# vllm-project/production-stack

Hardware: AMD Instinct MI355X
Metric: output_tokens_per_sec (higher is better)
Workload: dtype bfloat16; 1 GPU; multi-round-qa; model=llama-3-8b, users_per_gpu=320, rounds_per_conversation=10, max_model_len=8192, parallelism=dp1, prefix_caching=True, kv_cache_dtype=auto, quantization=none

## Files before the change

csrc/attention.hip:

```cpp
#include "ps_common.h"

template <int HEAD_DIM, int GQ, int BLOCK_SIZE, int NWAVES, int LOWREG,
          typename KVT>
__global__ __launch_bounds__(NWAVES * 64, LOWREG ? 3 : 1) void paged_attn_decode_kernel(
    unsigned short* __restrict__ out,
    float* __restrict__ ws_acc,
    float* __restrict__ ws_ml,
    const unsigned short* __restrict__ q,
    const KVT* __restrict__ k_cache,
    const KVT* __restrict__ v_cache,
    const int* __restrict__ block_tables,
    const int* __restrict__ seq_lens,
    int max_blocks, float scale, int KH, long q_stride, int window) {
  using KVTr = ps_kv_traits<KVT>;
  using kvec8 = typename KVTr::vec8;
  constexpr int D = HEAD_DIM;
  constexpr int LPG = D / 8;
  constexpr int TPW = 64 / LPG;
  static_assert(BLOCK_SIZE % TPW == 0, "block size must divide");

  const int seq = blockIdx.x;
  const int kvh = blockIdx.y;
  const int ctx = seq_lens[seq];
  const int wave = threadIdx.x >> 6;
  const int lane = threadIdx.x & 63;
  const int sg = lane / LPG;
  const int sl = lane % LPG;

  ps_bf16x8 qp[GQ];
  const unsigned short* qbase = q + (long)seq * q_stride + (long)kvh * GQ * D;
#pragma unroll
  for (int g = 0; g < GQ; g++)
    qp[g] = *(const ps_bf16x8*)(qbase + g * D + sl * 8);
  float qf[GQ][8];
  if constexpr (!LOWREG) {
#pragma unroll
    for (int g = 0; g < GQ; g++)
#pragma unroll
      for (int j = 0; j < 8; j++) qf[g][j] = ps_bf16_to_f32(qp[g][j]);
  }

  float m[GQ], l[GQ], acc[GQ][8];
#pragma unroll
  for (int g = 0; g < GQ; g++) {
    m[g] = PS_NEG_INF;
    l[g] = 0.f;
#pragma unroll
    for (int j = 0; j < 8; j++) acc[g][j] = 0.f;
  }

  const int nblocks = (ctx + BLOCK_SIZE - 1) / BLOCK_SIZE;
  const int win_lo = (window > 0 && ctx > window) ? ctx - window : 0;
  const int first_block = win_lo / BLOCK_SIZE;
  const int nsplit = gridDim.z;
  const int split = blockIdx.z;
  const int live_blocks = nblocks - first_block;
  const int per_split = (live_blocks + nsplit - 1) / nsplit;
  const int b_begin = first_block + split * per_split;
  const int b_end = min(nblocks, b_begin + per_split);
  const int* bt = block_tables + (long)seq * max_blocks;
  constexpr int TPB = BLOCK_SIZE / TPW;
  for (int b = b_begin + wave; b < b_end; b += NWAVES) {
    const long blk = bt[b];
    const KVT* kb = k_cache + ((blk * KH + kvh) * BLOCK_SIZE) * D;
    const KVT* vb = v_cache + ((blk * KH + kvh) * BLOCK_SIZE) * D;
    const int valid_tokens = min(BLOCK_SIZE, ctx - b * BLOCK_SIZE);
    float sc[GQ][TPB];
    kvec8 vv[TPB];
    if constexpr (LOWREG) {
#pragma unroll
      for (int g = 0; g < GQ; g++)
        asm volatile("" : "+v"(qp[g]));
    }
#pragma unroll
    for (int tt = 0; tt < TPB; tt++) {
      const int tok = tt * TPW + sg;
      const bool valid =
          tok < valid_tokens && b * BLOCK_SIZE + tok >= win_lo;
      kvec8 kv = *(const kvec8*)(kb + tok * D + sl * 8);
      if constexpr (!LOWREG)
        vv[tt] = *(const kvec8*)(vb + tok * D + sl * 8);
      float kf[8];
      KVTr::to_f32x8(kv, kf);
#pragma unroll
      for (int g = 0; g < GQ; g++) {
        float s = 0.f;
#pragma unroll
        for (int j = 0; j < 8; j++) {
          if constexpr (LOWREG)
            s += ps_bf16_to_f32(qp[g][j]) * kf[j];
          else
            s += qf[g][j] * kf[j];
        }
        s = ps_group_sum<LPG>(s) * scale;
        sc[g][tt] = valid ? s : PS_NEG_INF;
      }
    }
    if constexpr (LOWREG) {
#pragma unroll
      for (int tt = 0; tt < TPB; tt++)
        vv[tt] = *(const kvec8*)(vb + (tt * TPW + sg) * D + sl * 8);
    }
#pragma unroll
    for (int g = 0; g < GQ; g++) {
      float bmax = sc[g][0];
#pragma unroll
      for (int tt = 1; tt < TPB; tt++) bmax = fmaxf(bmax, sc[g][tt]);
      const float mnew = fmaxf(m[g], bmax);
      const float corr = __expf(m[g] - mnew);
      float p[TPB];
      float psum = 0.f;
#pragma unroll
// ... 18 lines not shown
#pragma unroll
  for (int off = LPG; off < 64; off <<= 1) {
#pragma unroll
    for (int g = 0; g < GQ; g++) {
      const float mo = __shfl_xor(m[g], off, 64);
      const float lo = __shfl_xor(l[g], off, 64);
      const float mnew = fmaxf(m[g], mo);
      const float c1 = __expf(m[g] - mnew);
      const float c2 = __expf(mo - mnew);
#pragma unroll
      for (int j = 0; j < 8; j++) {
        const float ao = __shfl_xor(acc[g][j], off, 64);
        acc[g][j] = acc[g][j] * c1 + ao * c2;
      }
      l[g] = l[g] * c1 + lo * c2;
      m[g] = mnew;
    }
  }

  __shared__ float sm[NWAVES][GQ];
  __shared__ float slse[NWAVES][GQ];
  __shared__ float sacc[NWAVES][GQ][D];
  if (sg == 0) {
#pragma unroll
    for (int g = 0; g < GQ; g++) {
      if (sl == 0) {
        sm[wave][g] = m[g];
        slse[wave][g] = l[g];
      }
#pragma unroll
      for (int j = 0; j < 8; j++) sacc[wave][g][sl * 8 + j] = acc[g][j];
    }
  }
  __syncthreads();
  if (wave == 0 && sg == 0) {
#pragma unroll
    for (int g = 0; g < GQ; g++) {
      float M = PS_NEG_INF, L = 0.f, A[8];
#pragma unroll
      for (int j = 0; j < 8; j++) A[j] = 0.f;
#pragma unroll
      for (int wv = 0; wv < NWAVES; wv++) {
        const float mw = sm[wv][g];
        const float mnew = fmaxf(M, mw);
        const float c1 = __expf(M - mnew);
        const float c2 = __expf(mw - mnew);
        L = L * c1 + slse[wv][g] * c2;
#pragma unroll
        for (int j = 0; j < 8; j++)
          A[j] = A[j] * c1 + sacc[wv][g][sl * 8 + j] * c2;
        M = mnew;
      }
      const long head = (long)seq * KH * GQ + (long)kvh * GQ + g;
      if (nsplit == 1) {
        const float inv = L > 0.f ? 1.f / L : 0.f;
        ps_bf16x8 ov;
#pragma unroll
        for (int j = 0; j < 8; j++) ov[j] = ps_f32_to_bf16(A[j] * inv);
        *(ps_bf16x8*)(out + head * D + sl * 8) = ov;
      } else {
        float* wa = ws_acc + (head * nsplit + split) * D + sl * 8;
#pragma unroll
        for (int j = 0; j < 8; j++) wa[j] = A[j];
        if (sl == 0) {
          float* wm = ws_ml + (head * nsplit + split) * 2;
          wm[0] = M;
          wm[1] = L;
        }
      }
    }
  }
}

template <int HEAD_DIM>
__global__ __launch_bounds__(64) void paged_attn_combine_kernel(
    unsigned short* __restrict__ out,
    const float* __restrict__ ws_acc,
    const float* __restrict__ ws_ml,
    int nsplit) {
  constexpr int D = HEAD_DIM;
  constexpr int LPG = D / 8;
  const long head = blockIdx.x;
  const int sl = threadIdx.x;
  if (sl >= LPG) return;
  float M = PS_NEG_INF, L = 0.f, A[8];
#pragma unroll
  for (int j = 0; j < 8; j++) A[j] = 0.f;
  for (int s = 0; s < nsplit; s++) {
    const float mw = ws_ml[(head * nsplit + s) * 2 + 0];
    const float lw = ws_ml[(head * nsplit + s) * 2 + 1];
    const float mnew = fmaxf(M, mw);
    const float c1 = __expf(M - mnew);
    const float c2 = __expf(mw - mnew);
    const float* wa = ws_acc + (head * nsplit + s) * D + sl * 8;
#pragma unroll
    for (int j = 0; j < 8; j++) A[j] = A[j] * c1 + wa[j] * c2;
    L = L * c1 + lw * c2;
    M = mnew;
  }
  const float inv = L > 0.f ? 1.f / L : 0.f;
  ps_bf16x8 ov;
#pragma unroll
  for (int j = 0; j < 8; j++) ov[j] = ps_f32_to_bf16(A[j] * inv);
  *(ps_bf16x8*)(out + head * D + sl * 8) = ov;
}

template <int HEAD_DIM, int BLOCK_SIZE>
__global__ __launch_bounds__(64) void paged_attn_prefill_kernel(
    unsigned short* __restrict__ out,
    const unsigned short* __restrict__ q,
    const unsigned short* __restrict__ k_cache,
    const unsigned short* __restrict__ v_cache,
    const int* __restrict__ block_tables,
    const int* __restrict__ token_seq,
    const int* __restrict__ token_pos,
    int max_blocks, float scale, int KH, int GQ, long q_stride,
    int window) {
  constexpr int D = HEAD_DIM;
  constexpr int LPG = D / 8;
  constexpr int TPW = 64 / LPG;

  const int tokid = blockIdx.x;
  const int qh = blockIdx.y;
  const int kvh = qh / GQ;
  const int seq = token_seq[tokid];
  const int pos = token_pos[tokid];
  const int ctx = pos + 1;
  const int lane = threadIdx.x & 63;
  const int sg = lane / LPG;
  const int sl = lane % LPG;
  const int QH = KH * GQ;

  float qf[8];
  {
    ps_bf16x8 qv =
        *(const ps_bf16x8*)(q + (long)tokid * q_stride + (long)qh * D + sl * 8);
#pragma unroll
    for (int j = 0; j < 8; j++) qf[j] = ps_bf16_to_f32(qv[j]) * scale;
  }

  float m = PS_NEG_INF, l = 0.f, acc[8];
#pragma unroll
  for (int j = 0; j < 8; j++) acc[j] = 0.f;

  const int nblocks = (ctx + BLOCK_SIZE - 1) / BLOCK_SIZE;
  const int win_lo = (window > 0 && ctx > window) ? ctx - window : 0;
  const int* bt = block_tables + (long)seq * max_blocks;
// ... 99 lines not shown
    for (int j = 0; j < 8; j++) {
      const float f = ps_bf16_to_f32(xv[j]);
      if (f > best) {
        best = f;
        besti = i + j;
      }
    }
  }
  const int tail_start = (V / 8) * 8;
  for (int i = tail_start + threadIdx.x; i < V; i += blockDim.x) {
    const float f = ps_bf16_to_f32(row[i]);
    if (f > best) {
      best = f;
      besti = i;
    }
  }
#pragma unroll
  for (int off = 32; off > 0; off >>= 1) {
    const float ob = __shfl_xor(best, off, 64);
    const int oi = __shfl_xor(besti, off, 64);
    if (ob > best || (ob == best && oi < besti)) {
      best = ob;
      besti = oi;
    }
  }
  __shared__ float wbest[4];
  __shared__ int wbesti[4];
  const int wave = threadIdx.x >> 6;
  if ((threadIdx.x & 63) == 0) {
    wbest[wave] = best;
    wbesti[wave] = besti;
  }
  __syncthreads();
  if (threadIdx.x == 0) {
    for (int wv = 1; wv < (int)(blockDim.x >> 6); wv++) {
      if (wbest[wv] > wbest[0] ||
          (wbest[wv] == wbest[0] && wbesti[wv] < wbesti[0])) {
        wbest[0] = wbest[wv];
        wbesti[0] = wbesti[wv];
      }
    }
    out[r] = wbesti[0];
  }
}

extern "C" {

int ps_paged_attn_decode(void* out, void* ws_acc, void* ws_ml, const void* q,
                         const void* k_cache, const void* v_cache,
                         const void* block_tables, const void* seq_lens,
                         int num_seqs, int max_blocks, float scale, int KH,
                         int GQ, int head_dim, int block_size, int num_splits,
                         long q_stride, int variant, int kv_fp8,
                         int window, hipStream_t stream) {
  dim3 grid(num_seqs, KH, num_splits);
  constexpr int NW = 4;
  dim3 block(NW * 64);
#define PS_DECODE_T(HD, G, BS, LR, KVT)                                      \
  paged_attn_decode_kernel<HD, G, BS, NW, LR, KVT>                           \
      <<<grid, block, 0, stream>>>(                                          \
          (unsigned short*)out, (float*)ws_acc, (float*)ws_ml,               \
          (const unsigned short*)q, (const KVT*)k_cache,                     \
          (const KVT*)v_cache, (const int*)block_tables,                     \
          (const int*)seq_lens, max_blocks, scale, KH, q_stride, window)
#define PS_DISPATCH_DECODE(HD, G, BS)                                        \
  do {                                                                       \
    if (kv_fp8) {                                                            \
      if (variant == 1)                                                      \
        PS_DECODE_T(HD, G, BS, 1, unsigned char);                            \
      else                                                                   \
        PS_DECODE_T(HD, G, BS, 0, unsigned char);                            \
    } else {                                                                 \
      if (variant == 1)                                                      \
        PS_DECODE_T(HD, G, BS, 1, unsigned short);                           \
      else                                                                   \
        PS_DECODE_T(HD, G, BS, 0, unsigned short);                           \
    }                                                                        \
    if (num_splits > 1)                                                      \
      paged_attn_combine_kernel<HD>                                          \
          <<<dim3(num_seqs * KH * G), 64, 0, stream>>>(                      \
              (unsigned short*)out, (const float*)ws_acc,                    \
              (const float*)ws_ml, num_splits);                              \
  } while (0)
  if (head_dim == 128 && block_size == 16) {
    switch (GQ) {
      case 1: PS_DISPATCH_DECODE(128, 1, 16); return 0;
      case 2: PS_DISPATCH_DECODE(128, 2, 16); return 0;
      case 3: PS_DISPATCH_DECODE(128, 3, 16); return 0;
      case 4: PS_DISPATCH_DECODE(128, 4, 16); return 0;
      case 6: PS_DISPATCH_DECODE(128, 6, 16); return 0;
      case 7: PS_DISPATCH_DECODE(128, 7, 16); return 0;
      case 8: PS_DISPATCH_DECODE(128, 8, 16); return 0;
      default: return -1;
    }
  }
  if (head_dim == 64 && block_size == 16 && !kv_fp8) {
    switch (GQ) {
      case 1: PS_DISPATCH_DECODE(64, 1, 16); return 0;
      case 2: PS_DISPATCH_DECODE(64, 2, 16); return 0;
      case 4: PS_DISPATCH_DECODE(64, 4, 16); return 0;
      case 8: PS_DISPATCH_DECODE(64, 8, 16); return 0;
      default: return -1;
    }
  }
  return -1;
#undef PS_DECODE_T
#undef PS_DISPATCH_DECODE
}

int ps_paged_attn_prefill(void* out, const void* q, const void* k_cache,
                          const void* v_cache, const void* block_tables,
                          const void* token_seq, const void* token_pos,
                          int num_tokens, int num_q_heads, int max_blocks,
                          float scale, int KH, int GQ, int head_dim,
                          int block_size, long q_stride, int window,
                          hipStream_t stream) {
  dim3 grid(num_tokens, num_q_heads);
  dim3 block(64);
#define PS_DISPATCH_PREFILL(HD, BS)                                         \
  paged_attn_prefill_kernel<HD, BS><<<grid, block, 0, stream>>>(            \
      (unsigned short*)out, (const unsigned short*)q,                       \
      (const unsigned short*)k_cache, (const unsigned short*)v_cache,       \
      (const int*)block_tables, (const int*)token_seq,                      \
      (const int*)token_pos, max_blocks, scale, KH, GQ, q_stride, window)
  if (head_dim == 128 && block_size == 16) {
    PS_DISPATCH_PREFILL(128, 16);
    return 0;
  }
  if (head_dim == 64 && block_size == 16) {
    PS_DISPATCH_PREFILL(64, 16);
    return 0;
  }
  return -1;
#undef PS_DISPATCH_PREFILL
}
// ... 29 lines not shown
```

csrc/bindings.cpp:

```cpp
#include <hip/hip_runtime.h>
#include <torch/extension.h>

#include <c10/hip/HIPStream.h>

#include <algorithm>

extern "C" {
void ps_rms_norm(void* out, const void* x, const void* w, float eps, long T,
                 int D, hipStream_t stream);
void ps_fused_add_rms_norm(void* x, void* residual, const void* w, float eps,
                           long T, int D, hipStream_t stream);
void ps_rms_norm_fp8(void* out_q, void* out_scale, void* x, void* residual,
                     const void* w, float eps, long T, int D, int fused,
                     hipStream_t stream);
void ps_silu_and_mul_fp8(void* out_q, void* out_scale, const void* x, long T,
                         int D, hipStream_t stream);
void ps_silu_and_mul(void* out, const void* x, long T, int D,
                     hipStream_t stream);
void ps_rope(const void* positions, void* q, void* k, const void* cos_sin,
             long T, int QH, int KH, int HD, int ROT, hipStream_t stream);
void ps_fused_rope_cache(void* qkv, const void* positions, const void* cos_sin,
                         const void* slot_mapping, void* k_cache,
                         void* v_cache, long T, int QH, int KH, int HD,
                         int ROT, long qkv_stride, int BS, int kv_fp8,
                         hipStream_t stream);
int ps_paged_attn_decode(void* out, void* ws_acc, void* ws_ml, const void* q,
                         const void* k_cache, const void* v_cache,
                         const void* block_tables, const void* seq_lens,
                         int num_seqs, int max_blocks, float scale, int KH,
                         int GQ, int head_dim, int block_size, int num_splits,
                         long q_stride, int variant, int kv_fp8, int window,
                         hipStream_t stream);
int ps_prefill_mfma32_splits(int num_tiles, int KH, int GQ);
int ps_paged_attn_prefill_mfma32(void* out, void* ws_o, void* ws_ml,
                                 long q_tokens, const void* q,
                                 const void* k_cache, const void* v_cache,
                                 const void* block_tables,
                                 const void* tile_info, int num_tiles,
                                 int num_q_heads, int max_blocks,
                                 float scale, int KH, int GQ, int head_dim,
                                 long q_stride, int kv_fp8, int window,
                                 hipStream_t stream);
int ps_paged_attn_prefill_mfma(void* out, const void* q, const void* k_cache,
                               const void* v_cache, const void* block_tables,
                               const void* tile_info, int num_tiles,
                               int num_q_heads, int max_blocks, float scale,
                               int KH, int GQ, int head_dim, long q_stride,
                               int variant, int kv_fp8, int window, hipStream_t stream);
int ps_paged_attn_prefill(void* out, const void* q, const void* k_cache,
                          const void* v_cache, const void* block_tables,
                          const void* token_seq, const void* token_pos,
                          int num_tokens, int num_q_heads, int max_blocks,
                          float scale, int KH, int GQ, int head_dim,
                          int block_size, long q_stride, int window,
                          hipStream_t stream);
void ps_reshape_and_cache(const void* k, const void* v, void* k_cache,
                          void* v_cache, const void* slot_mapping, long T,
                          int KH, int HD, int BS, int kv_fp8,
                          hipStream_t stream);
void ps_greedy_sample(void* out, const void* logits, long R, int V,
                      hipStream_t stream);
void ps_kv_quant(void* out, void* scales, const void* in, long rows, int hd,
                 hipStream_t stream);
void ps_kv_dequant(void* out, const void* in, const void* scales, long rows,
                   int hd, hipStream_t stream);
int ps_skinny_gemm_splits(int M, int N, int K);
int ps_skinny_gemm(void* out_bf16, void* ws, const void* x, const void* w,
                   int M, int N, int K, long x_stride, hipStream_t stream);
int ps_gemm8p_splits(int M, int N, int K);
int ps_gemm8p(void* out_bf16, void* ws, const void* x, const void* w, int M,
              int N, int K, long x_stride, hipStream_t stream);
int ps_lora_bgmv(void* out, const void* x, const void* A, const void* B,
                 const void* scale, const void* idx, int T, int IN, int W,
                 int R, long out_stride, long x_stride, int col_off,
                 hipStream_t stream);
}

at::Tensor cachegen_encode(at::Tensor q);
at::Tensor cachegen_decode(at::Tensor blob, int64_t hd);

namespace {

hipStream_t current_stream() {
  return c10::hip::getCurrentHIPStream().stream();
}
// ... 22 lines not shown
  TORCH_CHECK(q.dim() == 3 && q.stride(2) == 1 && q.stride(1) == HD,
              "q must be [T, H, HD] with contiguous heads");
  return q.stride(0);
}

void rms_norm(at::Tensor out, at::Tensor x, at::Tensor w, double eps) {
  CHECK_GPU_BF16(out);
  CHECK_GPU_BF16(x);
  CHECK_GPU_BF16(w);
  const long T = x.numel() / x.size(-1);
  const int D = (int)x.size(-1);
  TORCH_CHECK(D % 8 == 0, "hidden dim must be a multiple of 8");
  ps_rms_norm(out.data_ptr(), x.data_ptr(), w.data_ptr(), (float)eps, T, D,
              current_stream());
}

void fused_add_rms_norm(at::Tensor x, at::Tensor residual, at::Tensor w,
                        double eps) {
  CHECK_GPU_BF16(x);
  CHECK_GPU_BF16(residual);
  CHECK_GPU_BF16(w);
  const long T = x.numel() / x.size(-1);
  const int D = (int)x.size(-1);
  TORCH_CHECK(D % 8 == 0, "hidden dim must be a multiple of 8");
  ps_fused_add_rms_norm(x.data_ptr(), residual.data_ptr(), w.data_ptr(),
                        (float)eps, T, D, current_stream());
}

void silu_and_mul(at::Tensor out, at::Tensor x) {
  CHECK_GPU_BF16(out);
  CHECK_GPU_BF16(x);
  const int D = (int)out.size(-1);
  TORCH_CHECK(x.size(-1) == 2 * D, "x last dim must be 2*out last dim");
  TORCH_CHECK(D % 8 == 0, "feature dim must be a multiple of 8");
  const long T = out.numel() / D;
  ps_silu_and_mul(out.data_ptr(), x.data_ptr(), T, D, current_stream());
}

void rotary_embedding(at::Tensor positions, at::Tensor q, at::Tensor k,
                      at::Tensor cos_sin, long head_dim) {
  CHECK_GPU_DTYPE(positions, at::kInt);
  CHECK_GPU_BF16(q);
  CHECK_GPU_BF16(k);
  CHECK_GPU_DTYPE(cos_sin, at::kFloat);
  const long T = positions.size(0);
  const int HD = (int)head_dim;
  const int ROT = (int)cos_sin.size(-1);
  const int QH = (int)(q.numel() / T / HD);
  const int KH = (int)(k.numel() / T / HD);
  ps_rope(positions.data_ptr(), q.data_ptr(), k.data_ptr(),
          cos_sin.data_ptr(), T, QH, KH, HD, ROT, current_stream());
}

void paged_attn_decode(at::Tensor out, at::Tensor q, at::Tensor k_cache,
                       at::Tensor v_cache, at::Tensor block_tables,
                       at::Tensor seq_lens, double scale, int64_t num_splits,
                       int64_t variant, int64_t window) {
  CHECK_GPU_BF16(out);
  const int kv_fp8 = cache_fp8(k_cache);
  cache_fp8(v_cache);
  CHECK_GPU_DTYPE(block_tables, at::kInt);
  CHECK_GPU_DTYPE(seq_lens, at::kInt);
  const int S = (int)q.size(0);
  const int QH = (int)q.size(1);
  const int HD = (int)q.size(2);
  const int KH = (int)k_cache.size(1);
  const int BS = (int)k_cache.size(2);
  TORCH_CHECK(QH % KH == 0, "GQA group mismatch");
  const int GQ = QH / KH;
  const int max_blocks = (int)block_tables.size(1);
  if (num_splits <= 0) {
    const int target = 2048;
    num_splits = std::min<int64_t>(
        32, std::max<int64_t>(1, target / std::max(1, S * KH)));
  }
  at::Tensor ws_acc, ws_ml;
  void *acc_p = nullptr, *ml_p = nullptr;
  if (num_splits > 1) {
    auto opts = q.options().dtype(at::kFloat);
    ws_acc = at::empty({(long)S * QH * num_splits * HD}, opts);
    ws_ml = at::empty({(long)S * QH * num_splits * 2}, opts);
    acc_p = ws_acc.data_ptr();
    ml_p = ws_ml.data_ptr();
  }
  int rc = ps_paged_attn_decode(
      out.data_ptr(), acc_p, ml_p, q.data_ptr(), k_cache.data_ptr(),
      v_cache.data_ptr(), block_tables.data_ptr(), seq_lens.data_ptr(), S,
      max_blocks, (float)scale, KH, GQ, HD, BS, (int)num_splits,
      q_row_stride(q, HD), (int)variant, kv_fp8, (int)window,
      current_stream());
  TORCH_CHECK(rc == 0, "unsupported decode config: head_dim=", HD,
              " block_size=", BS, " gqa=", GQ);
}

void paged_attn_prefill(at::Tensor out, at::Tensor q, at::Tensor k_cache,
                        at::Tensor v_cache, at::Tensor block_tables,
                        at::Tensor token_seq, at::Tensor token_pos,
                        double scale, int64_t window) {
  CHECK_GPU_BF16(out);
  CHECK_GPU_BF16(k_cache);
  CHECK_GPU_BF16(v_cache);
  CHECK_GPU_DTYPE(block_tables, at::kInt);
  CHECK_GPU_DTYPE(token_seq, at::kInt);
  CHECK_GPU_DTYPE(token_pos, at::kInt);
  const int T = (int)q.size(0);
  const int QH = (int)q.size(1);
  const int HD = (int)q.size(2);
  const int KH = (int)k_cache.size(1);
  const int BS = (int)k_cache.size(2);
  TORCH_CHECK(QH % KH == 0, "GQA group mismatch");
  const int GQ = QH / KH;
  const int max_blocks = (int)block_tables.size(1);
  int rc = ps_paged_attn_prefill(
      out.data_ptr(), q.data_ptr(), k_cache.data_ptr(), v_cache.data_ptr(),
      block_tables.data_ptr(), token_seq.data_ptr(), token_pos.data_ptr(), T,
      QH, max_blocks, (float)scale, KH, GQ, HD, BS, q_row_stride(q, HD),
      (int)window, current_stream());
  TORCH_CHECK(rc == 0, "unsupported prefill config: head_dim=", HD,
              " block_size=", BS);
}

void paged_attn_prefill_mfma(at::Tensor out, at::Tensor q,
                             at::Tensor k_cache, at::Tensor v_cache,
                             at::Tensor block_tables, at::Tensor tile_info,
                             double scale, int64_t variant, int64_t window) {
  CHECK_GPU_BF16(out);
  const int kv_fp8 = cache_fp8(k_cache);
  cache_fp8(v_cache);
  CHECK_GPU_DTYPE(block_tables, at::kInt);
  CHECK_GPU_DTYPE(tile_info, at::kInt);
  const int QH = (int)q.size(1);
  const int HD = (int)q.size(2);
  const int KH = (int)k_cache.size(1);
  TORCH_CHECK(QH % KH == 0, "GQA group mismatch");
  TORCH_CHECK(k_cache.size(2) == 16, "mfma prefill needs block_size 16");
  const int GQ = QH / KH;
  const int NT = (int)tile_info.size(0);
  int rc;
  if (variant == 5) {
    const int splits = ps_prefill_mfma32_splits(NT, KH, QH / KH);
    const long T = q.size(0);
    void *ws_o_p = nullptr, *ws_ml_p = nullptr;
    at::Tensor ws_o, ws_ml;
// ... 159 lines not shown
  TORCH_CHECK(out.size(0) == T && idx.numel() == T, "T mismatch");
  TORCH_CHECK(col_off + W <= out.size(1), "col range out of bounds");
  int rc = ps_lora_bgmv(out.data_ptr(), x.data_ptr(), A.data_ptr(),
                        B.data_ptr(), scale.data_ptr(), idx.data_ptr(), T,
                        IN, W, R, out.stride(0), x.stride(0), (int)col_off,
                        current_stream());
  TORCH_CHECK(rc == 0, "lora_bgmv unsupported (R>64?) R=", R);
}

void kv_quant(at::Tensor out, at::Tensor scales, at::Tensor in) {
  CHECK_GPU_DTYPE(out, at::kChar);
  CHECK_GPU_DTYPE(scales, at::kFloat);
  CHECK_GPU_BF16(in);
  const int hd = (int)in.size(-1);
  TORCH_CHECK(hd % 8 == 0, "row width must be multiple of 8");
  const long rows = in.numel() / hd;
  ps_kv_quant(out.data_ptr(), scales.data_ptr(), in.data_ptr(), rows, hd,
              current_stream());
}

void kv_dequant(at::Tensor out, at::Tensor in, at::Tensor scales) {
  CHECK_GPU_BF16(out);
  CHECK_GPU_DTYPE(in, at::kChar);
  CHECK_GPU_DTYPE(scales, at::kFloat);
  const int hd = (int)out.size(-1);
  const long rows = out.numel() / hd;
  ps_kv_dequant(out.data_ptr(), in.data_ptr(), scales.data_ptr(), rows, hd,
                current_stream());
}

void greedy_sample(at::Tensor out, at::Tensor logits) {
  CHECK_GPU_DTYPE(out, at::kLong);
  CHECK_GPU_BF16(logits);
  const long R = logits.size(0);
  const int V = (int)logits.size(1);
  ps_greedy_sample(out.data_ptr(), logits.data_ptr(), R, V, current_stream());
}

}

PYBIND11_MODULE(TORCH_EXTENSION_NAME, m) {
  m.def("rms_norm", &rms_norm, "RMSNorm (bf16)");
  m.def("fused_add_rms_norm", &fused_add_rms_norm,
        "Fused residual add + RMSNorm (bf16, in-place)");
  m.def("silu_and_mul", &silu_and_mul, "SiLU-and-mul (bf16)");
  m.def("rotary_embedding", &rotary_embedding,
        "Neox-style rotary embedding (bf16, in-place)");
  m.def("paged_attn_decode", &paged_attn_decode,
        "Paged attention, decode phase (bf16 KV, split-KV)",
        pybind11::arg("out"), pybind11::arg("q"), pybind11::arg("k_cache"),
        pybind11::arg("v_cache"), pybind11::arg("block_tables"),
        pybind11::arg("seq_lens"), pybind11::arg("scale"),
        pybind11::arg("num_splits") = 0, pybind11::arg("variant") = 0,
        pybind11::arg("window") = 0);
  m.def("paged_attn_prefill", &paged_attn_prefill,
        "Paged attention, chunked prefill (bf16 KV)");
  m.def("lora_bgmv", &lora_bgmv,
        "batched-grouped LoRA matvec (per-token adapter slots)");
  m.def("paged_attn_prefill_mfma", &paged_attn_prefill_mfma,
        "Paged attention, chunked prefill via MFMA tiles (head_dim 128)",
        pybind11::arg("out"), pybind11::arg("q"), pybind11::arg("k_cache"),
        pybind11::arg("v_cache"), pybind11::arg("block_tables"),
        pybind11::arg("tile_info"), pybind11::arg("scale"),
        pybind11::arg("variant") = 4, pybind11::arg("window") = 0);
  m.def("fused_rope_cache", &fused_rope_cache,
        "Fused RoPE + paged KV append on the packed qkv tensor");
  m.def("reshape_and_cache", &reshape_and_cache,
        "Append K/V for new tokens into the paged cache");
  m.def("greedy_sample", &greedy_sample, "Per-row argmax over vocab");
  m.def("kv_quant", &kv_quant, "Row-wise int8 KV quantization");
  m.def("rms_norm_fp8", &rms_norm_fp8,
        "RMSNorm (optionally fused residual add) emitting fp8 + row scales");
  m.def("silu_and_mul_fp8", &silu_and_mul_fp8,
        "SiLU-mul emitting fp8 + row scales");
  m.def("cachegen_encode", &cachegen_encode,
        "CacheGen-style adaptive range encode of int8 KV (CPU)");
  m.def("cachegen_decode", &cachegen_decode,
        "CacheGen-style range decode -> int8 (CPU)");
  m.def("gemm8p", &gemm8p,
        "8-phase deep-pipelined bf16 GEMM (out = x @ w.T)");
  m.def("skinny_gemm", &skinny_gemm,
        "Split-K MFMA GEMM for decode-shaped (M<=128) projections");
  m.def("kv_dequant", &kv_dequant, "Row-wise int8 KV dequantization");
}
```

production_stack_amd/engine/models/llama.py:

```python

from __future__ import annotations

import math
from typing import List, Optional

import torch
import torch.nn as nn
import torch.nn.functional as F

from production_stack_amd import ops
from production_stack_amd.ops import gemm_policy
from production_stack_amd.engine.config import ModelConfig
from production_stack_amd.parallel import state as pstate


class BatchMeta:

    def __init__(
        self,
        positions: torch.Tensor,
        slot_mapping: torch.Tensor,
        num_prefill_tokens: int,
        prefill_token_seq: Optional[torch.Tensor],
        prefill_token_pos: Optional[torch.Tensor],
# ... 124 lines not shown
                residual = hidden
                hidden = ops.rms_norm(hidden, self.input_norm,
                                      cfg.rms_norm_eps)
            else:
                hidden, residual = ops.fused_add_rms_norm(
                    hidden, residual, self.input_norm, cfg.rms_norm_eps
                )
            if fp8 is not None:
                qkv = ops.fp8_linear(hidden, *fp8["qkv"])
            else:
                qkv = gemm_policy.linear(hidden, self.qkv_proj)
        if self.qkv_bias is not None:
            qkv = qkv + self.qkv_bias
        qs = self.q_heads * self.head_dim
        kvs = self.kv_heads * self.head_dim
        slots = getattr(self, "lora_slots", None)
        if slots is not None and meta.lora_idx is not None:
            li = self.layer_idx
            slots.apply("q", li, qkv, hidden, meta.lora_idx)
            slots.apply("k", li, qkv, hidden, meta.lora_idx)
            slots.apply("v", li, qkv, hidden, meta.lora_idx)
        elif meta.lora_groups:
            from production_stack_amd.engine.lora import apply_lora_slice

            li = self.layer_idx
            apply_lora_slice(qkv, hidden, meta.lora_groups, li, "q", 0, qs)
            apply_lora_slice(qkv, hidden, meta.lora_groups, li, "k", qs, kvs)
            apply_lora_slice(
                qkv, hidden, meta.lora_groups, li, "v", qs + kvs, kvs
            )
        T = qkv.shape[0]
        k_cache, v_cache = kv_cache
        if qkv.is_cuda:
            ops.fused_rope_cache(
                qkv, meta.positions, cos_sin, meta.slot_mapping,
                k_cache, v_cache, self.q_heads, self.head_dim,
            )
            qh = qkv.view(T, -1, self.head_dim)[:, : self.q_heads]
        else:
            q = qkv[:, :qs].contiguous()
            k = qkv[:, qs : qs + kvs].contiguous()
            v = qkv[:, qs + kvs :].contiguous()
            q, k = ops.rotary_embedding(
                meta.positions, q, k, cos_sin, self.head_dim
            )
            ops.reshape_and_cache(
                k.view(T, self.kv_heads, self.head_dim),
                v.view(T, self.kv_heads, self.head_dim),
                k_cache,
                v_cache,
                meta.slot_mapping,
            )
            qh = q.view(T, self.q_heads, self.head_dim)
        outs: List[torch.Tensor] = []
        tp = meta.num_prefill_tokens
        if tp > 0:
            if (
                qh.is_cuda
                and self.head_dim == 128
                and meta.prefill_tiles is not None
            ):
                outs.append(
                    ops.paged_attn_prefill_mfma(
                        qh[:tp],
                        k_cache,
                        v_cache,
                        meta.prefill_block_tables,
                        meta.prefill_tiles,
                        self.scale,
                        self.window,
                    )
                )
            else:
                outs.append(
                    ops.paged_attn_prefill(
                        qh[:tp] if qh.is_cuda else qh[:tp].contiguous(),
                        k_cache,
                        v_cache,
                        meta.prefill_block_tables,
                        meta.prefill_token_seq,
                        meta.prefill_token_pos,
                        self.scale,
                        self.window,
                    )
                )
        if meta.num_decode_seqs > 0:
            outs.append(
                ops.paged_attn_decode(
                    qh[tp:] if qh.is_cuda else qh[tp:].contiguous(),
                    k_cache,
                    v_cache,
                    meta.decode_block_tables,
                    meta.decode_seq_lens,
                    self.scale,
                    self.window,
                )
            )
        attn = torch.cat(outs, dim=0) if len(outs) > 1 else outs[0]
        if getattr(self, "fp8_w", None) is not None:
            attn_out = ops.fp8_linear(attn.reshape(T, qs),
                                      *self.fp8_w["o"])
        else:
            attn_out = gemm_policy.linear(attn.view(T, qs), self.o_proj)
        if slots is not None and meta.lora_idx is not None:
            slots.apply("o", self.layer_idx, attn_out,
                        attn.reshape(T, qs), meta.lora_idx)
        elif meta.lora_groups:
            apply_lora_slice(
                attn_out, attn.view(T, qs), meta.lora_groups,
                self.layer_idx, "o",
            )
        attn_out = pstate.tp_all_reduce(attn_out)

        if self.n_experts:
            hidden, residual = ops.fused_add_rms_norm(
                attn_out, residual, self.post_attn_norm, cfg.rms_norm_eps
            )
            mlp_out = self._moe_forward(hidden)
            mlp_out = pstate.tp_all_reduce(mlp_out)
            return mlp_out, residual
        if fuse_q:
            xq, sx = ops.rms_norm_fp8(
                attn_out, self.post_attn_norm, cfg.rms_norm_eps,
                residual=residual)
            hidden = attn_out
            gate_up = ops.fp8_linear_rowwise(xq, sx, *fp8["gate_up"])
        else:
            hidden, residual = ops.fused_add_rms_norm(
                attn_out, residual, self.post_attn_norm, cfg.rms_norm_eps
            )
            if fp8 is not None:
                gate_up = ops.fp8_linear(hidden, *fp8["gate_up"])
            else:
                gate_up = gemm_policy.linear(hidden, self.gate_up_proj)
        if slots is not None and meta.lora_idx is not None:
            slots.apply("gate", self.layer_idx, gate_up, hidden,
                        meta.lora_idx)
            slots.apply("up", self.layer_idx, gate_up, hidden,
                        meta.lora_idx)
        elif meta.lora_groups:
            apply_lora_slice(
                gate_up, hidden, meta.lora_groups, self.layer_idx,
                "gate", 0, self.inter,
            )
            apply_lora_slice(
                gate_up, hidden, meta.lora_groups, self.layer_idx,
                "up", self.inter, self.inter,
            )
        if fuse_q:
            aq, sa = ops.silu_and_mul_fp8(gate_up)
            act = gate_up[:, : self.inter]
# ... 167 lines not shown
```

production_stack_amd/ops/__init__.py:

```python

from __future__ import annotations

import os

import torch

from production_stack_amd.ops import reference

try:
    from production_stack_amd import _C
except ImportError:
    _C = None

HAVE_EXT = _C is not None


def _require_ext() -> None:
    if _C is None:
        raise RuntimeError(
            "production_stack_amd._C HIP extension is not built; run "
            "`PYTORCH_ROCM_ARCH=gfx950 python setup.py build_ext --inplace`. "
            "Refusing to fall back to eager PyTorch on GPU."
        )

# ... 26 lines not shown
        _C.silu_and_mul(out, x)
        return out
    return reference.silu_and_mul(x)


def rotary_embedding(
    positions: torch.Tensor,
    q: torch.Tensor,
    k: torch.Tensor,
    cos_sin: torch.Tensor,
    head_dim: int,
) -> tuple[torch.Tensor, torch.Tensor]:
    if q.is_cuda:
        _require_ext()
        _C.rotary_embedding(positions, q, k, cos_sin, head_dim)
        return q, k
    return reference.rotary_embedding(positions, q, k, cos_sin, head_dim)


def fused_rope_cache(
    qkv: torch.Tensor,
    positions: torch.Tensor,
    cos_sin: torch.Tensor,
    slot_mapping: torch.Tensor,
    k_cache: torch.Tensor,
    v_cache: torch.Tensor,
    q_heads: int,
    head_dim: int,
) -> None:
    _require_ext()
    _C.fused_rope_cache(
        qkv, positions, cos_sin, slot_mapping, k_cache, v_cache, q_heads,
        head_dim,
    )


def reshape_and_cache(
    k: torch.Tensor,
    v: torch.Tensor,
    k_cache: torch.Tensor,
    v_cache: torch.Tensor,
    slot_mapping: torch.Tensor,
) -> None:
    if k_cache.is_cuda:
        _require_ext()
        _C.reshape_and_cache(
            k.view(k.shape[0], -1), v.view(v.shape[0], -1), k_cache, v_cache,
            slot_mapping,
        )
        return
    reference.reshape_and_cache(k, v, k_cache, v_cache, slot_mapping)


def paged_attn_decode(
    q: torch.Tensor,
    k_cache: torch.Tensor,
    v_cache: torch.Tensor,
    block_tables: torch.Tensor,
    seq_lens: torch.Tensor,
    scale: float,
    window: int = 0,
) -> torch.Tensor:
    if q.is_cuda:
        _require_ext()
        out = torch.empty(q.shape, dtype=q.dtype, device=q.device)
        _C.paged_attn_decode(
            out, q, k_cache, v_cache, block_tables, seq_lens, scale, 0, 1,
            window
        )
        return out
    return reference.paged_attn_decode(
        q, k_cache, v_cache, block_tables, seq_lens, scale, window
    )


def paged_attn_prefill(
    q: torch.Tensor,
    k_cache: torch.Tensor,
    v_cache: torch.Tensor,
    block_tables: torch.Tensor,
    token_seq: torch.Tensor,
    token_pos: torch.Tensor,
    scale: float,
    window: int = 0,
) -> torch.Tensor:
    if q.is_cuda:
        _require_ext()
        out = torch.empty(q.shape, dtype=q.dtype, device=q.device)
        _C.paged_attn_prefill(
            out, q, k_cache, v_cache, block_tables, token_seq, token_pos,
            scale, window
        )
        return out
    return reference.paged_attn_prefill(
        q, k_cache, v_cache, block_tables, token_seq, token_pos, scale,
        window
    )


PREFILL_VARIANT = int(os.environ.get("PS_PREFILL_VARIANT", "5"))


def prefill_tile_rows(num_q_heads: int, num_kv_heads: int) -> int:
    if PREFILL_VARIANT != 5:
        return 64
    gq = max(1, num_q_heads // max(1, num_kv_heads))
    gqw = 1
    while gqw < 4 and gq % (gqw * 2) == 0:
        gqw *= 2
    return 32 * (8 // gqw)


def paged_attn_prefill_mfma(
    q: torch.Tensor,
    k_cache: torch.Tensor,
    v_cache: torch.Tensor,
    block_tables: torch.Tensor,
    tile_info: torch.Tensor,
    scale: float,
    window: int = 0,
    variant: int = None,
) -> torch.Tensor:
    _require_ext()
    out = torch.empty(q.shape, dtype=q.dtype, device=q.device)
    v = PREFILL_VARIANT if variant is None else variant
    _C.paged_attn_prefill_mfma(
        out, q, k_cache, v_cache, block_tables, tile_info, scale, v, window
    )
    return out


def greedy_sample(logits: torch.Tensor) -> torch.Tensor:
    if logits.is_cuda:
        _require_ext()
        if logits.dtype != torch.bfloat16:
            return logits.float().argmax(dim=-1)
        out = torch.empty(
            logits.shape[0], dtype=torch.long, device=logits.device
        )
        _C.greedy_sample(out, logits)
        return out
    return reference.greedy_sample(logits)


def kv_quant(x: torch.Tensor) -> tuple:
    if x.is_cuda:
        _require_ext()
        hd = x.shape[-1]
        out = torch.empty(x.shape, dtype=torch.int8, device=x.device)
        scales = torch.empty(
            x.numel() // hd, dtype=torch.float32, device=x.device
        )
        _C.kv_quant(out, scales, x)
        return out, scales
    return reference.kv_quant(x)


def kv_dequant(
    q: torch.Tensor, scales: torch.Tensor, dtype=torch.bfloat16
) -> torch.Tensor:
    if q.is_cuda:
        _require_ext()
        out = torch.empty(q.shape, dtype=dtype, device=q.device)
        _C.kv_dequant(out, q, scales)
        return out
    return reference.kv_dequant(q, scales, dtype)


def skinny_gemm(x: torch.Tensor, w: torch.Tensor) -> torch.Tensor:
    _require_ext()
    out = torch.empty(
        (x.shape[0], w.shape[0]), dtype=torch.bfloat16, device=x.device
    )
    _C.skinny_gemm(out, x, w)
    return out


# ... 124 lines not shown
```

Baseline: 5623 tokens/s.

## Use fixed-size context chunks for decode split-K and write attention outputs in place

```diff
diff --git a/csrc/attention.hip b/csrc/attention.hip
--- a/csrc/attention.hip
+++ b/csrc/attention.hip
@@ -11,7 +11,8 @@
     const KVT* __restrict__ v_cache,
     const int* __restrict__ block_tables,
     const int* __restrict__ seq_lens,
-    int max_blocks, float scale, int KH, long q_stride, int window) {
+    int max_blocks, float scale, int KH, long q_stride, int window,
+    int chunk_blocks) {
   using KVTr = ps_kv_traits<KVT>;
   using kvec8 = typename KVTr::vec8;
   constexpr int D = HEAD_DIM;
@@ -22,42 +23,54 @@
   const int seq = blockIdx.x;
   const int kvh = blockIdx.y;
   const int ctx = seq_lens[seq];
-  const int wave = threadIdx.x >> 6;
-  const int lane = threadIdx.x & 63;
-  const int sg = lane / LPG;
-  const int sl = lane % LPG;
-
-  ps_bf16x8 qp[GQ];
-  const unsigned short* qbase = q + (long)seq * q_stride + (long)kvh * GQ * D;
-#pragma unroll
-  for (int g = 0; g < GQ; g++)
-    qp[g] = *(const ps_bf16x8*)(qbase + g * D + sl * 8);
-  float qf[GQ][8];
-  if constexpr (!LOWREG) {
-#pragma unroll
-    for (int g = 0; g < GQ; g++)
-#pragma unroll
-      for (int j = 0; j < 8; j++) qf[g][j] = ps_bf16_to_f32(qp[g][j]);
-  }
-
-  float m[GQ], l[GQ], acc[GQ][8];
-#pragma unroll
-  for (int g = 0; g < GQ; g++) {
-    m[g] = PS_NEG_INF;
-    l[g] = 0.f;
-#pragma unroll
-    for (int j = 0; j < 8; j++) acc[g][j] = 0.f;
-  }
-
   const int nblocks = (ctx + BLOCK_SIZE - 1) / BLOCK_SIZE;
   const int win_lo = (window > 0 && ctx > window) ? ctx - window : 0;
   const int first_block = win_lo / BLOCK_SIZE;
   const int nsplit = gridDim.z;
   const int split = blockIdx.z;
   const int live_blocks = nblocks - first_block;
-  const int per_split = (live_blocks + nsplit - 1) / nsplit;
-  const int b_begin = first_block + split * per_split;
-  const int b_end = min(nblocks, b_begin + per_split);
+  int b_begin, b_end;
+  bool direct;
+  if (chunk_blocks > 0) {
+    const int nchunk =
+        max(1, (live_blocks + chunk_blocks - 1) / chunk_blocks);
+    if (split >= nchunk) return;
+    b_begin = first_block + split * chunk_blocks;
+    b_end = min(nblocks, b_begin + chunk_blocks);
+    direct = nchunk == 1;
+  } else {
+    const int per_split = (live_blocks + nsplit - 1) / nsplit;
+    b_begin = first_block + split * per_split;
+    b_end = min(nblocks, b_begin + per_split);
+    direct = nsplit == 1;
+  }
+  const int wave = threadIdx.x >> 6;
+  const int lane = threadIdx.x & 63;
+  const int sg = lane / LPG;
+  const int sl = lane % LPG;
+
+  ps_bf16x8 qp[GQ];
+  const unsigned short* qbase = q + (long)seq * q_stride + (long)kvh * GQ * D;
+#pragma unroll
+  for (int g = 0; g < GQ; g++)
+    qp[g] = *(const ps_bf16x8*)(qbase + g * D + sl * 8);
+  float qf[GQ][8];
+  if constexpr (!LOWREG) {
+#pragma unroll
+    for (int g = 0; g < GQ; g++)
+#pragma unroll
+      for (int j = 0; j < 8; j++) qf[g][j] = ps_bf16_to_f32(qp[g][j]);
+  }
+
+  float m[GQ], l[GQ], acc[GQ][8];
+#pragma unroll
+  for (int g = 0; g < GQ; g++) {
+    m[g] = PS_NEG_INF;
+    l[g] = 0.f;
+#pragma unroll
+    for (int j = 0; j < 8; j++) acc[g][j] = 0.f;
+  }
+
   const int* bt = block_tables + (long)seq * max_blocks;
   constexpr int TPB = BLOCK_SIZE / TPW;
   for (int b = b_begin + wave; b < b_end; b += NWAVES) {
@@ -182,16 +195,17 @@
         M = mnew;
       }
       const long head = (long)seq * KH * GQ + (long)kvh * GQ + g;
-      if (nsplit == 1) {
+      if (direct) {
         const float inv = L > 0.f ? 1.f / L : 0.f;
         ps_bf16x8 ov;
 #pragma unroll
         for (int j = 0; j < 8; j++) ov[j] = ps_f32_to_bf16(A[j] * inv);
         *(ps_bf16x8*)(out + head * D + sl * 8) = ov;
       } else {
-        float* wa = ws_acc + (head * nsplit + split) * D + sl * 8;
-#pragma unroll
-        for (int j = 0; j < 8; j++) wa[j] = A[j];
+        float4* wa =
+            (float4*)(ws_acc + (head * nsplit + split) * D + sl * 8);
+        wa[0] = make_float4(A[0], A[1], A[2], A[3]);
+        wa[1] = make_float4(A[4], A[5], A[6], A[7]);
         if (sl == 0) {
           float* wm = ws_ml + (head * nsplit + split) * 2;
           wm[0] = M;
@@ -207,22 +221,35 @@
     unsigned short* __restrict__ out,
     const float* __restrict__ ws_acc,
     const float* __restrict__ ws_ml,
-    int nsplit) {
+    int nsplit, const int* __restrict__ seq_lens, int QH, int block_size,
+    int window, int chunk_blocks) {
   constexpr int D = HEAD_DIM;
   constexpr int LPG = D / 8;
   const long head = blockIdx.x;
   const int sl = threadIdx.x;
   if (sl >= LPG) return;
+  int nlive = nsplit;
+  if (chunk_blocks > 0) {
+    const int ctx = seq_lens[head / QH];
+    const int nblocks = (ctx + block_size - 1) / block_size;
+    const int win_lo = (window > 0 && ctx > window) ? ctx - window : 0;
+    const int live_blocks = nblocks - win_lo / block_size;
+    nlive = (live_blocks + chunk_blocks - 1) / chunk_blocks;
+    if (nlive <= 1) return;
+  }
   float M = PS_NEG_INF, L = 0.f, A[8];
 #pragma unroll
   for (int j = 0; j < 8; j++) A[j] = 0.f;
-  for (int s = 0; s < nsplit; s++) {
+  for (int s = 0; s < nlive; s++) {
     const float mw = ws_ml[(head * nsplit + s) * 2 + 0];
     const float lw = ws_ml[(head * nsplit + s) * 2 + 1];
     const float mnew = fmaxf(M, mw);
     const float c1 = __expf(M - mnew);
     const float c2 = __expf(mw - mnew);
-    const float* wa = ws_acc + (head * nsplit + s) * D + sl * 8;
+    const float4* wp =
+        (const float4*)(ws_acc + (head * nsplit + s) * D + sl * 8);
+    const float4 w0 = wp[0], w1 = wp[1];
+    const float wa[8] = {w0.x, w0.y, w0.z, w0.w, w1.x, w1.y, w1.z, w1.w};
 #pragma unroll
     for (int j = 0; j < 8; j++) A[j] = A[j] * c1 + wa[j] * c2;
     L = L * c1 + lw * c2;
@@ -428,9 +455,10 @@
                          int num_seqs, int max_blocks, float scale, int KH,
                          int GQ, int head_dim, int block_size, int num_splits,
                          long q_stride, int variant, int kv_fp8,
-                         int window, hipStream_t stream) {
+                         int window, int chunk_blocks, hipStream_t stream) {
   dim3 grid(num_seqs, KH, num_splits);
   constexpr int NW = 4;
+  if (chunk_blocks < 0 || chunk_blocks % NW != 0) return -2;
   dim3 block(NW * 64);
 #define PS_DECODE_T(HD, G, BS, LR, KVT)                                      \
   paged_attn_decode_kernel<HD, G, BS, NW, LR, KVT>                           \
@@ -438,7 +466,8 @@
           (unsigned short*)out, (float*)ws_acc, (float*)ws_ml,               \
           (const unsigned short*)q, (const KVT*)k_cache,                     \
           (const KVT*)v_cache, (const int*)block_tables,                     \
-          (const int*)seq_lens, max_blocks, scale, KH, q_stride, window)
+          (const int*)seq_lens, max_blocks, scale, KH, q_stride, window,     \
+          chunk_blocks)
 #define PS_DISPATCH_DECODE(HD, G, BS)                                        \
   do {                                                                       \
     if (kv_fp8) {                                                            \
@@ -456,7 +485,8 @@
       paged_attn_combine_kernel<HD>                                          \
           <<<dim3(num_seqs * KH * G), 64, 0, stream>>>(                      \
               (unsigned short*)out, (const float*)ws_acc,                    \
-              (const float*)ws_ml, num_splits);                              \
+              (const float*)ws_ml, num_splits, (const int*)seq_lens,         \
+              KH * G, BS, window, chunk_blocks);                             \
   } while (0)
   if (head_dim == 128 && block_size == 16) {
     switch (GQ) {
diff --git a/csrc/bindings.cpp b/csrc/bindings.cpp
--- a/csrc/bindings.cpp
+++ b/csrc/bindings.cpp
@@ -30,7 +30,7 @@
                          int num_seqs, int max_blocks, float scale, int KH,
                          int GQ, int head_dim, int block_size, int num_splits,
                          long q_stride, int variant, int kv_fp8, int window,
-                         hipStream_t stream);
+                         int chunk_blocks, hipStream_t stream);
 int ps_prefill_mfma32_splits(int num_tiles, int KH, int GQ);
 int ps_paged_attn_prefill_mfma32(void* out, void* ws_o, void* ws_ml,
                                  long q_tokens, const void* q,
@@ -159,10 +159,14 @@
           cos_sin.data_ptr(), T, QH, KH, HD, ROT, current_stream());
 }
 
+constexpr int kDecodeChunkMinWork = 2048;
+constexpr int kDecodeChunkBlocks = 128;
+
 void paged_attn_decode(at::Tensor out, at::Tensor q, at::Tensor k_cache,
                        at::Tensor v_cache, at::Tensor block_tables,
                        at::Tensor seq_lens, double scale, int64_t num_splits,
-                       int64_t variant, int64_t window) {
+                       int64_t variant, int64_t window,
+                       int64_t chunk_blocks) {
   CHECK_GPU_BF16(out);
   const int kv_fp8 = cache_fp8(k_cache);
   cache_fp8(v_cache);
@@ -176,11 +180,20 @@
   TORCH_CHECK(QH % KH == 0, "GQA group mismatch");
   const int GQ = QH / KH;
   const int max_blocks = (int)block_tables.size(1);
-  if (num_splits <= 0) {
-    const int target = 2048;
-    num_splits = std::min<int64_t>(
-        32, std::max<int64_t>(1, target / std::max(1, S * KH)));
+  TORCH_CHECK(chunk_blocks >= 0 && chunk_blocks % 4 == 0,
+              "chunk_blocks must be a non-negative multiple of 4");
+  if (chunk_blocks == 0 && num_splits <= 0) {
+    if (S * KH >= kDecodeChunkMinWork) {
+      chunk_blocks = kDecodeChunkBlocks;
+    } else {
+      const int target = 2048;
+      num_splits = std::min<int64_t>(
+          32, std::max<int64_t>(1, target / std::max(1, S * KH)));
+    }
   }
+  if (chunk_blocks > 0)
+    num_splits = std::max<int64_t>(
+        1, (max_blocks + chunk_blocks - 1) / chunk_blocks);
   at::Tensor ws_acc, ws_ml;
   void *acc_p = nullptr, *ml_p = nullptr;
   if (num_splits > 1) {
@@ -195,7 +208,7 @@
       v_cache.data_ptr(), block_tables.data_ptr(), seq_lens.data_ptr(), S,
       max_blocks, (float)scale, KH, GQ, HD, BS, (int)num_splits,
       q_row_stride(q, HD), (int)variant, kv_fp8, (int)window,
-      current_stream());
+      (int)chunk_blocks, current_stream());
   TORCH_CHECK(rc == 0, "unsupported decode config: head_dim=", HD,
               " block_size=", BS, " gqa=", GQ);
 }
@@ -461,7 +474,7 @@
         pybind11::arg("v_cache"), pybind11::arg("block_tables"),
         pybind11::arg("seq_lens"), pybind11::arg("scale"),
         pybind11::arg("num_splits") = 0, pybind11::arg("variant") = 0,
-        pybind11::arg("window") = 0);
+        pybind11::arg("window") = 0, pybind11::arg("chunk_blocks") = 0);
   m.def("paged_attn_prefill", &paged_attn_prefill,
         "Paged attention, chunked prefill (bf16 KV)");
   m.def("lora_bgmv", &lora_bgmv,
diff --git a/production_stack_amd/engine/models/llama.py b/production_stack_amd/engine/models/llama.py
--- a/production_stack_amd/engine/models/llama.py
+++ b/production_stack_amd/engine/models/llama.py
@@ -200,7 +200,9 @@
                 meta.slot_mapping,
             )
             qh = q.view(T, self.q_heads, self.head_dim)
-        outs: List[torch.Tensor] = []
+        attn = torch.empty(
+            (T, self.q_heads, self.head_dim), dtype=qh.dtype, device=qh.device
+        )
         tp = meta.num_prefill_tokens
         if tp > 0:
             if (
@@ -208,43 +210,39 @@
                 and self.head_dim == 128
                 and meta.prefill_tiles is not None
             ):
-                outs.append(
-                    ops.paged_attn_prefill_mfma(
-                        qh[:tp],
-                        k_cache,
-                        v_cache,
-                        meta.prefill_block_tables,
-                        meta.prefill_tiles,
-                        self.scale,
-                        self.window,
-                    )
-                )
-            else:
-                outs.append(
-                    ops.paged_attn_prefill(
-                        qh[:tp] if qh.is_cuda else qh[:tp].contiguous(),
-                        k_cache,
-                        v_cache,
-                        meta.prefill_block_tables,
-                        meta.prefill_token_seq,
-                        meta.prefill_token_pos,
-                        self.scale,
-                        self.window,
-                    )
-                )
-        if meta.num_decode_seqs > 0:
-            outs.append(
-                ops.paged_attn_decode(
-                    qh[tp:] if qh.is_cuda else qh[tp:].contiguous(),
+                ops.paged_attn_prefill_mfma(
+                    qh[:tp],
                     k_cache,
                     v_cache,
-                    meta.decode_block_tables,
-                    meta.decode_seq_lens,
+                    meta.prefill_block_tables,
+                    meta.prefill_tiles,
                     self.scale,
                     self.window,
-                )
-            )
-        attn = torch.cat(outs, dim=0) if len(outs) > 1 else outs[0]
+                    out=attn[:tp],
+                )
+            else:
+                ops.paged_attn_prefill(
+                    qh[:tp] if qh.is_cuda else qh[:tp].contiguous(),
+                    k_cache,
+                    v_cache,
+                    meta.prefill_block_tables,
+                    meta.prefill_token_seq,
+                    meta.prefill_token_pos,
+                    self.scale,
+                    self.window,
+                    out=attn[:tp],
+                )
+        if meta.num_decode_seqs > 0:
+            ops.paged_attn_decode(
+                qh[tp:] if qh.is_cuda else qh[tp:].contiguous(),
+                k_cache,
+                v_cache,
+                meta.decode_block_tables,
+                meta.decode_seq_lens,
+                self.scale,
+                self.window,
+                out=attn[tp:],
+            )
         if getattr(self, "fp8_w", None) is not None:
             attn_out = ops.fp8_linear(attn.reshape(T, qs),
                                       *self.fp8_w["o"])
diff --git a/production_stack_amd/ops/__init__.py b/production_stack_amd/ops/__init__.py
--- a/production_stack_amd/ops/__init__.py
+++ b/production_stack_amd/ops/__init__.py
@@ -102,6 +102,26 @@
     reference.reshape_and_cache(k, v, k_cache, v_cache, slot_mapping)
 
 
+DECODE_POLICY = os.environ.get("PS_DECODE_POLICY", "balanced")
+if DECODE_POLICY not in ("balanced", "legacy"):
+    raise ValueError(
+        f"PS_DECODE_POLICY must be 'balanced' or 'legacy', "
+        f"got {DECODE_POLICY!r}"
+    )
+
+
+def decode_num_splits(num_seqs: int, num_kv_heads: int) -> int:
+    if DECODE_POLICY == "legacy":
+        return min(32, max(1, 2048 // max(1, num_seqs * num_kv_heads)))
+    return 0
+
+
+def _check_out(out: torch.Tensor, q: torch.Tensor) -> torch.Tensor:
+    if out.shape != q.shape or out.dtype != q.dtype or out.device != q.device:
+        raise ValueError("out must match q's shape, dtype and device")
+    return out
+
+
 def paged_attn_decode(
     q: torch.Tensor,
     k_cache: torch.Tensor,
@@ -110,18 +130,26 @@
     seq_lens: torch.Tensor,
     scale: float,
     window: int = 0,
+    out: torch.Tensor = None,
 ) -> torch.Tensor:
     if q.is_cuda:
         _require_ext()
-        out = torch.empty(q.shape, dtype=q.dtype, device=q.device)
+        if out is None:
+            out = torch.empty(q.shape, dtype=q.dtype, device=q.device)
+        else:
+            _check_out(out, q)
         _C.paged_attn_decode(
-            out, q, k_cache, v_cache, block_tables, seq_lens, scale, 0, 1,
-            window
-        )
-        return out
-    return reference.paged_attn_decode(
+            out, q, k_cache, v_cache, block_tables, seq_lens, scale,
+            decode_num_splits(q.shape[0], k_cache.shape[1]), 1, window
+        )
+        return out
+    res = reference.paged_attn_decode(
         q, k_cache, v_cache, block_tables, seq_lens, scale, window
     )
+    if out is None:
+        return res
+    _check_out(out, q).copy_(res)
+    return out
 
 
 def paged_attn_prefill(
@@ -133,19 +161,27 @@
     token_pos: torch.Tensor,
     scale: float,
     window: int = 0,
+    out: torch.Tensor = None,
 ) -> torch.Tensor:
     if q.is_cuda:
         _require_ext()
-        out = torch.empty(q.shape, dtype=q.dtype, device=q.device)
+        if out is None:
+            out = torch.empty(q.shape, dtype=q.dtype, device=q.device)
+        else:
+            _check_out(out, q)
         _C.paged_attn_prefill(
             out, q, k_cache, v_cache, block_tables, token_seq, token_pos,
             scale, window
         )
         return out
-    return reference.paged_attn_prefill(
+    res = reference.paged_attn_prefill(
         q, k_cache, v_cache, block_tables, token_seq, token_pos, scale,
         window
     )
+    if out is None:
+        return res
+    _check_out(out, q).copy_(res)
+    return out
 
 
 PREFILL_VARIANT = int(os.environ.get("PS_PREFILL_VARIANT", "5"))
@@ -170,9 +206,13 @@
     scale: float,
     window: int = 0,
     variant: int = None,
-) -> torch.Tensor:
-    _require_ext()
-    out = torch.empty(q.shape, dtype=q.dtype, device=q.device)
+    out: torch.Tensor = None,
+) -> torch.Tensor:
+    _require_ext()
+    if out is None:
+        out = torch.empty(q.shape, dtype=q.dtype, device=q.device)
+    else:
+        _check_out(out, q)
     v = PREFILL_VARIANT if variant is None else variant
     _C.paged_attn_prefill_mfma(
         out, q, k_cache, v_cache, block_tables, tile_info, scale, v, window
```

Result: no change. 5593 tokens/s (-0.5%).
